# adamnelsonarcher/BB-OCR

Measured on AMD Instinct MI355X. Metric: book-page images/sec end-to-end (detect+recognize) @1280x960, higher is better.
Workload: dtype fp16

## Files before the change

### bb-ocr_amd/csrc/conv_mfma.hip

```cpp
#include "common.h"
#include "kernels.h"
#include <type_traits>
#include <utility>

__device__ __forceinline__ void lds_dma16(const void* gptr, const void* lds) {
    const unsigned la = (unsigned)(size_t)(const __attribute__((address_space(3))) void*)lds;
    asm volatile("s_mov_b32 m0, %1\n\ts_nop 0\n\tglobal_load_lds_dwordx4 %0, off" ::"v"(gptr), "s"(la) : "memory");
}

template <int EL, int MF, bool ADDUP = false>
__device__ __forceinline__ void conv_epilogue(const ConvArgs& a, f32x4 (&acc)[MF][4], int n, int nt, int oy0, int ox0, int wm, int wn, int fpr,
                                              int lane, int BN, int sub = 1, int sph = 0, int spw = 0) {
    const int g = lane >> 4, pl = lane & 15;
    const int cout0 = nt * BN + wn * 64 + g * 8;
    if (a.tail) {
        const float* tw = a.tail;
        const typename El<EL>::v8 w1f = *(const typename El<EL>::v8*)(a.tail_frag + lane * 8);
        float cb[8], b1r[4], w2a[4], w2b[4];
#pragma unroll
        for (int i = 0; i < 8; ++i) cb[i] = a.bias[(g & 1) * 8 + i];
#pragma unroll
        for (int r = 0; r < 4; ++r) { b1r[r] = tw[4 * g + r]; w2a[r] = tw[16 + 4 * g + r]; w2b[r] = tw[32 + 4 * g + r]; }
        const float b20 = tw[48], b21 = tw[49];
#pragma unroll
// ... 421 lines not shown
    const int n_wi = a.NP >> 4;
    const int l_pix = (lane & 7) + ((lane >> 5) << 3);
    const int l_kg = (lane >> 3) & 3;
    int src_pix[PITER];
#pragma unroll
    for (int it = 0; it < PITER; ++it) {
        const int wi = wave + it * NW;
        int sp = -1;
        if (wi < n_wi) {
            const int pix = wi * 16 + l_pix;
            const int py = pix / a.PW, px = pix - py * a.PW;
            const int iy = iy0 + py, ix = ix0 + px;
            if (py < a.PH && iy >= 0 && iy < a.H && ix >= 0 && ix < a.W) sp = (n * a.H + iy) * a.W + ix;
        }
        src_pix[it] = sp;
    }
    constexpr int NPART = (PITER + 3) / 4, PH = PITER / NPART;
    u32x4 pre[PH];
    auto load_part = [&](int chunk, auto part_c) {
        constexpr int part = decltype(part_c)::value;
        const int c = chunk * 32;
        const bool s0 = c < a.C0;
        const uint16_t* src = s0 ? a.in0 : a.in1;
        const int cs = s0 ? a.in0_cs : a.in1_cs;
        const int cb = (s0 ? c : c - a.C0) + l_kg * 8;
#pragma unroll
        for (int i = 0; i < PH; ++i) {
            const int sp = src_pix[part * PH + i];
            u32x4 v = {0u, 0u, 0u, 0u};
            if (sp >= 0) v = *(const u32x4*)(src + (size_t)sp * cs + cb);
            pre[i] = v;
        }
    };
    auto store_part = [&](int chunk, auto part_c) {
        constexpr int part = decltype(part_c)::value;
        unsigned char* pb = pbuf + (chunk & 1) * patch_bytes;
        const bool relu = (chunk * 32 < a.C0) ? a.relu_in0 : a.relu_in1;
#pragma unroll
        for (int i = 0; i < PH; ++i) {
            const int wi = wave + (part * PH + i) * NW;
            if (wi < n_wi) {
                u32x4 v = pre[i];
                if (relu) {
                    const s16x8 z = {0, 0, 0, 0, 0, 0, 0, 0};
                    v = __builtin_bit_cast(u32x4, __builtin_elementwise_max(__builtin_bit_cast(s16x8, v), z));
                }
                *(u32x4*)(pb + (size_t)(l_kg * a.NP + wi * 16 + l_pix) * 16) = v;
            }
        }
    };
    using P0 = std::integral_constant<int, 0>;
    const int S = (a.ntaps - 1) / NPART;
    auto stage_patch_load = [&](int chunk, int tap) {
        if (tap == 0) load_part(chunk, P0{});
        if constexpr (NPART > 1) { if (tap == S) load_part(chunk, std::integral_constant<int, (NPART > 1 ? 1 : 0)>{}); }
        if constexpr (NPART > 2) { if (tap == 2 * S) load_part(chunk, std::integral_constant<int, (NPART > 2 ? 2 : 0)>{}); }
        if constexpr (NPART > 3) { if (tap == 3 * S) load_part(chunk, std::integral_constant<int, (NPART > 3 ? 3 : 0)>{}); }
    };
    auto stage_patch_store = [&](int chunk, int tap) {
        if (tap == S - 1) store_part(chunk, P0{});
        if constexpr (NPART > 1) { if (tap == 2 * S - 1) store_part(chunk, std::integral_constant<int, (NPART > 1 ? 1 : 0)>{}); }
        if constexpr (NPART > 2) { if (tap == 3 * S - 1) store_part(chunk, std::integral_constant<int, (NPART > 2 ? 2 : 0)>{}); }
        if constexpr (NPART > 3) { if (tap == 4 * S - 1) store_part(chunk, std::integral_constant<int, (NPART > 3 ? 3 : 0)>{}); }
    };
    auto stage_patch_now = [&](int chunk) {
        load_part(chunk, P0{});
        store_part(chunk, P0{});
        if constexpr (NPART > 1) { load_part(chunk, std::integral_constant<int, (NPART > 1 ? 1 : 0)>{}); store_part(chunk, std::integral_constant<int, (NPART > 1 ? 1 : 0)>{}); }
        if constexpr (NPART > 2) { load_part(chunk, std::integral_constant<int, (NPART > 2 ? 2 : 0)>{}); store_part(chunk, std::integral_constant<int, (NPART > 2 ? 2 : 0)>{}); }
        if constexpr (NPART > 3) { load_part(chunk, std::integral_constant<int, (NPART > 3 ? 3 : 0)>{}); store_part(chunk, std::integral_constant<int, (NPART > 3 ? 3 : 0)>{}); }
    };
    const unsigned char* wsrc = (const unsigned char*)a.wpk + (size_t)nt * nk * WBUF;
    auto issue_w = [&](int ks, int buf) {
#pragma unroll
        for (int p0 = 0; p0 < WPIECES; p0 += NT) {
            if (p0 + wave * 64 < WPIECES) {
                __builtin_amdgcn_global_load_lds(
                    (const __attribute__((address_space(1))) void*)(wsrc + (size_t)ks * WBUF + (size_t)(p0 + tid) * 16),
                    (__attribute__((address_space(3))) void*)(wbuf + buf * WBUF + (p0 + wave * 64) * 16), 16, 0, 0);
            }
        }
    };

    const int fpr = a.TW >> 4;
    int frag_off[MF];
#pragma unroll
    for (int f = 0; f < MF; ++f) {
        const int F = wm * MF + f;
        const int fr = F / fpr, fc = F - fr * fpr;
        frag_off[f] = (fr * a.PW + fc * 16) * 16;
    }
    const int lane_patch_off = ((lane >> 4) * a.NP + (lane & 15)) * 16;
    const int lane_w_off = wn * 4 * 1024 + lane * 16;

    f32x4 acc[MF][4];
#pragma unroll
    for (int f = 0; f < MF; ++f)
#pragma unroll
        for (int j = 0; j < 4; ++j) acc[f][j] = (f32x4){0.f, 0.f, 0.f, 0.f};

    {
        issue_w(0, 0);
        stage_patch_now(0);
        __syncthreads();
        int ks = 0;
        for (int c = 0; c < a.nchunks; ++c) {
            const bool more = (c + 1 < a.nchunks);
            if (more && a.ntaps < 3) load_part(c + 1, P0{});
            const unsigned char* pbase = pbuf + (c & 1) * patch_bytes + lane_patch_off;
            int ky = 0, kx = 0;
            for (int tap = 0; tap < a.ntaps; ++tap, ++ks) {
                if (more && a.ntaps >= 3) stage_patch_load(c + 1, tap);
                if (ks + 1 < nk) issue_w(ks + 1, (ks + 1) & 1);
                const unsigned char* wb = wbuf + (ks & 1) * WBUF + lane_w_off;
                typename El<EL>::v8 af[4];
#pragma unroll
                for (int j = 0; j < 4; ++j) af[j] = *(const typename El<EL>::v8*)(wb + j * 1024);
                const unsigned char* pb = pbase + ((ky * a.PW + kx) * a.dil) * 16;
                typename El<EL>::v8 bq[MF];
#pragma unroll
                for (int f = 0; f < MF; ++f) bq[f] = *(const typename El<EL>::v8*)(pb + frag_off[f]);
#pragma unroll
                for (int f = 0; f < MF; ++f) {
#pragma unroll
                    for (int j = 0; j < 4; ++j) acc[f][j] = El<EL>::mfma(af[j], bq[f], acc[f][j]);
                }
                __builtin_amdgcn_sched_group_barrier(0x100, 4 + MF, 0);
                __builtin_amdgcn_sched_group_barrier(0x008, 4 * MF, 0);
                if (more) {
                    if (a.ntaps >= 3) stage_patch_store(c + 1, tap);
                    else if (tap == a.ntaps - 1) store_part(c + 1, P0{});
                }
                __syncthreads();
                if (++kx == a.KW) { kx = 0; ++ky; }
            }
        }
    }

    conv_epilogue<EL, MF>(a, acc, n, nt, oy0, ox0, wm, wn, fpr, lane, BN);
}

template <int EL, int WM, int WN, int MF, int NPB, int RING, int NPS = NPB * 64, bool FUSE1 = false, int NF = 4, int EPI = 0, int KS = 3>
__global__ void __launch_bounds__(WM * WN * 64, 2) conv3x3_dma_kernel(const ConvArgs a) {
    constexpr int NTAP = KS * KS, PAD = KS == 3 ? 1 : 0;
    static_assert((KS == 3 || KS == 2) && (KS == 3 || (!FUSE1 && EPI == 0)), "kernel size");
    constexpr int NW = WM * WN, NT = NW * 64, BN = WN * 64;
    static_assert(NW == 4, "one wave per 8-channel group of the patch");
    constexpr int WBUF = BN * 64, WPIECES = WBUF / 16, WPT = WPIECES / NT;
    static_assert(WPIECES % NT == 0 && (RING == 3 || RING == 4), "uniform DMA issue");
    constexpr int NP = NPS, PSLOTS = NTAP + 1 - RING;
    constexpr int PPER = (NPB + PSLOTS - 1) / PSLOTS;
    static_assert(NPS <= NPB * 64 && NPS > (NPB - 1) * 64 && NPS % 4 == 0, "patch size");
    static_assert(PSLOTS >= 1 && PPER * PSLOTS >= NPB, "patch does not fit the DMA schedule");
    extern __shared__ __attribute__((aligned(16))) unsigned char smem[];
    unsigned char* const wbuf = smem;
    unsigned char* const pbuf = smem + RING * WBUF;
    constexpr int patch_bytes = NP * 64;

    const int tid = threadIdx.x;
    const int lane = tid & 63;
    const int wave = __builtin_amdgcn_readfirstlane(tid >> 6);
    const int wm = wave / WN, wn = wave % WN;
    const int sub = a.sub;
    const int nk = a.nchunks * NTAP;
    const int fpr = FUSE1 ? 1 : a.TW >> 4;
    const int PW = FUSE1 ? 18 : a.PW;

    const int tile = xcd_remap(blockIdx.x, gridDim.x);
    struct Geo {
        int n, nt, oy0, ox0, sph, spw;
        const unsigned char* wsrc;
    };
    auto geom = [&](int id, Geo& g) {
        g.nt = id % a.ntiles_n;
        id /= a.ntiles_n;
        const int tx = id % a.tiles_x;
        id /= a.tiles_x;
        const int ty = id % a.tiles_y;
        int n = id / a.tiles_y;
        g.sph = 0; g.spw = 0;
        g.n = n;
        g.oy0 = ty * a.TH; g.ox0 = tx * a.TW;
        g.wsrc = (const unsigned char*)a.wpk + (size_t)g.nt * nk * WBUF;
    };
    int spix[NPB];
    const int pw_magic = (65536 + a.PW - 1) / a.PW;
    const int stack_magic = ((1 << 20) + a.stack) / (a.stack + 1);
    auto geom_pix = [&](const Geo& g) {
        const int iy0 = g.oy0 - PAD, ix0 = g.ox0 - PAD;
#pragma unroll
        for (int pb = 0; pb < NPB; ++pb) {
            const int pix = pb * 64 + lane;
            const int py = (pix * pw_magic) >> 16, px = pix - py * a.PW;
            int ly = iy0 + py;
            const int lx = ix0 + px;
            int sph = 0, spw = 0;
            bool rowok = ly >= 0;
            if (sub > 1) {
                const int vy = ly < 0 ? 0 : ly;
                const int q = (vy * stack_magic) >> 20;
                ly = vy - q * (a.stack + 1);
                sph = q / sub;
                spw = q - sph * sub;
                rowok = rowok && ly < a.stack && q < sub * sub;
            }
            const int iy = ly * sub + sph, ix = lx * sub + spw;
            spix[pb] = (py < a.PH && rowok && iy < a.H && lx >= 0 && ix < a.W) ? (g.n * a.H + iy) * a.W + ix : -1;
        }
    };
    Geo cur;
    geom(tile, cur);
    if constexpr (!FUSE1) geom_pix(cur);

    auto issue_p = [&](int sp, int chunk, int par, auto pb_c) {
        constexpr int pb = decltype(pb_c)::value;
        const int c = chunk * 32;
        const bool s0 = c < a.C0;
        const uint16_t* src = s0 ? a.in0 : a.in1;
        const int cs = s0 ? a.in0_cs : a.in1_cs;
        const int cb = (s0 ? c : c - a.C0) + wave * 8;
        const uint16_t* gp = sp >= 0 ? src + (size_t)sp * cs + cb : (const uint16_t*)a.zero;
        if ((pb + 1) * 64 <= NPS || pb * 64 + lane < NPS)
            lds_dma16(gp, pbuf + par * patch_bytes + (wave * NP + pb * 64) * 16);
    };
    auto issue_w = [&](const unsigned char* slice, int slot) {
#pragma unroll
        for (int p0 = 0; p0 < WPIECES; p0 += NT) lds_dma16(slice + (size_t)(p0 + tid) * 16, wbuf + slot * WBUF + (p0 + wave * 64) * 16);
    };
    int frag_off[MF];
#pragma unroll
    for (int f = 0; f < MF; ++f) {
        const int F = wm * MF + f;
        const int fr = F / fpr, fc = F - fr * fpr;
        frag_off[f] = (fr * PW + fc * 16) * 16;
    }
    const int lane_patch_off = ((lane >> 4) * NP + (lane & 15)) * 16;
    const int lane_w_off = wn * 4 * 1024 + lane * 16;

    struct Sched {
        static constexpr int pcnt(int tap) {
            if (FUSE1 || tap >= PSLOTS) return 0;
            const int base = NPB / PSLOTS, extra = NPB % PSLOTS;
            return base + (tap < extra ? 1 : 0);
        }
        static constexpr int pfirst(int tap) { int s = 0; for (int t = 0; t < tap; ++t) s += pcnt(t); return s; }
        static constexpr int wcnt(bool more, int tap) { return (more || tap < NTAP - (RING - 1)) ? WPT : 0; }
        static constexpr int younger(bool more, int tap) {
            int nv = wcnt(more, tap) + (more ? pcnt(tap) : 0);
            for (int back = 1; back <= RING - 2; ++back) {
                const int t = tap - back;
                const bool m = t >= 0 ? more : true;
                const int tt = t >= 0 ? t : t + NTAP;
                const int pc = m ? pcnt(tt) : 0;
                nv += (back == RING - 2) ? pc : (wcnt(m, tt) + pc);
            }
            return nv;
        }
    };
    static_assert(FUSE1 || Sched::pfirst(NTAP) == NPB, "patch DMA schedule must cover the patch");

#pragma unroll
    for (int i = 0; i < RING - 1; ++i)
        if (i < nk) issue_w(cur.wsrc + (size_t)i * WBUF, i);
    if constexpr (!FUSE1) {
        [&]<int... PB>(std::integer_sequence<int, PB...>) { (issue_p(spix[PB], 0, 0, std::integral_constant<int, PB>{}), ...); }(std::make_integer_sequence<int, NPB>{});
    } else {
        static_assert(!FUSE1 || (RING == 3 && BN == 64 && NPS == 324), "fused conv1_1 producer: 16x16 tiles, 3-deep ring of 4 KB slices");
        u32x2* const rgbp = (u32x2*)(wbuf + 2 * WBUF);
        const uint8_t* rgb = (const uint8_t*)a.in0;
        const float m0 = 0.485f * 255.0f, m1 = 0.456f * 255.0f, m2 = 0.406f * 255.0f;
        const float s0 = 0.229f * 255.0f, s1 = 0.224f * 255.0f, s2 = 0.225f * 255.0f;
        static_assert(NT == 256, "two patch pixels per thread");
        int pq[2];
        bool on_canvas[2];
        unsigned int cr[2], cg[2], cb[2];
#pragma unroll
        for (int it = 0; it < 2; ++it) {
            const int p = tid + it * NT;
            const int py = p / 20, px = p - py * 20;
            const int iy = cur.oy0 - 2 + py, ix = cur.ox0 - 2 + px;
            pq[it] = p;
            on_canvas[it] = p < 400 && iy >= 0 && iy < a.H && ix >= 0 && ix < a.W;
            const bool on_page = on_canvas[it] && iy < a.rgb_H && ix < a.rgb_W;
            const uint8_t* q = rgb + (on_page ? ((size_t)(cur.n * a.rgb_H + iy) * a.rgb_W + ix) * 3 : (size_t)cur.n * a.rgb_H * a.rgb_W * 3);
            cr[it] = q[0]; cg[it] = q[1]; cb[it] = q[2];
            if (!on_page) { cr[it] = 0u; cg[it] = 0u; cb[it] = 0u; }
        }
        typename El<EL>::v8 w1[4];
#pragma unroll
        for (int j = 0; j < 4; ++j) w1[j] = *(const typename El<EL>::v8*)(a.c11_w + ((size_t)j * 64 + lane) * 8);
        const int g = lane >> 4, pl = lane & 15;
        f32x4 b1[4];
#pragma unroll
        for (int h = 0; h < 2; ++h)
#pragma unroll
            for (int q4 = 0; q4 < 2; ++q4) b1[h * 2 + q4] = *(const f32x4*)(a.c11_b + h * 32 + g * 8 + q4 * 4);
        __builtin_amdgcn_sched_barrier(0);
#pragma unroll
        for (int it = 0; it < 2; ++it) {
            if (pq[it] < 400) {
                u32x2 v = {0u, 0u};
                if (on_canvas[it]) {
                    v[0] = El<EL>::pack2(((float)cr[it] - m0) / s0, ((float)cg[it] - m1) / s1);
                    v[1] = El<EL>::pack2(((float)cb[it] - m2) / s2, 0.f);
                }
                rgbp[pq[it]] = v;
            }
        }
        __syncthreads();
        auto frag_geo = [&](int fi, int& pp, int& py, int& px) {
            pp = fi * 16 + pl;
            py = pp / 18;
            px = pp - py * 18;
        };
#pragma unroll
        for (int b3 = 0; b3 < 2; ++b3) {
            typename El<EL>::v8 bfr[3];
            int pps[3], pys[3], pxs[3];
#pragma unroll
            for (int q = 0; q < 3; ++q) {
                const int fi = wave + (b3 * 3 + q) * NW;
                frag_geo(fi < 21 ? fi : 20, pps[q], pys[q], pxs[q]);
                const int pc = pps[q] < 324 ? pys[q] * 20 + pxs[q] : 0;
                const int t0 = 2 * g, t1 = t0 + 1;
                const u32x2 a0 = rgbp[pc + (t0 / 3) * 20 + (t0 % 3)];
                const u32x2 a1 = rgbp[pc + (t1 / 3) * 20 + (t1 % 3)];
                const u32x2 t8 = rgbp[pc + 2 * 20 + 2];
                const unsigned int x = g == 0 ? (t8[0] << 16) : (g == 1 ? (t8[1] << 16) : 0u);
                const unsigned int y = g == 0 ? (t8[0] & 0xffff0000u) : 0u;
                bfr[q] = __builtin_bit_cast(typename El<EL>::v8, (u32x4){a0[0], a0[1] | x, a1[0], a1[1] | y});
            }
            f32x4 d[3][4];
#pragma unroll
            for (int q = 0; q < 3; ++q)
#pragma unroll
                for (int j = 0; j < 4; ++j) d[q][j] = El<EL>::mfma(w1[j], bfr[q], b1[j]);
#pragma unroll
            for (int q = 0; q < 3; ++q) {
                const int fi = wave + (b3 * 3 + q) * NW;
                const int pp = pps[q];
                const int iy = cur.oy0 - 1 + pys[q], ix = cur.ox0 - 1 + pxs[q];
                const bool inside = iy >= 0 && iy < a.H && ix >= 0 && ix < a.W;
                const float cap = inside ? __builtin_inff() : 0.f;
                if (fi < 21 && pp < 324) {
#pragma unroll
                    for (int h = 0; h < 2; ++h) {
                        u32x4 o;
#pragma unroll
                        for (int i = 0; i < 4; ++i) {
                            const int k = h * 8 + i * 2;
                            const float x0 = __builtin_amdgcn_fmed3f(d[q][k >> 2][k & 3], 0.f, cap), x1 = __builtin_amdgcn_fmed3f(d[q][(k + 1) >> 2][(k + 1) & 3], 0.f, cap);
                            o[i] = El<EL>::pack2(x0, x1);
                        }
                        *(u32x4*)(pbuf + h * patch_bytes + (g * NP + pp) * 16) = o;
                    }
                }
            }
        }
    }
    asm volatile("s_waitcnt vmcnt(0) lgkmcnt(0)\n\ts_barrier" ::: "memory");

    int wslot = 0, par = 0;
    const unsigned char* wp = cur.wsrc + (size_t)(RING - 1) * WBUF;
    f32x4 acc[MF][4];
#pragma unroll
    for (int f = 0; f < MF; ++f)
#pragma unroll
        for (int j = 0; j < 4; ++j) acc[f][j] = (f32x4){0.f, 0.f, 0.f, 0.f};
    static_assert(MF % 2 == 0 && MF >= 4, "B fragments are scheduled in pairs, four ahead");
    typename El<EL>::v8 pre[4];
    auto step = [&](auto tap_c, auto more_c, int c) {
        constexpr int tap = decltype(tap_c)::value;
        constexpr bool MORE = decltype(more_c)::value;
        constexpr int ky = tap / KS, kx = tap % KS;
        const unsigned char* wb = wbuf + wslot * WBUF + lane_w_off;
        const unsigned char* pb = pbuf + par * patch_bytes + lane_patch_off + (ky * PW + kx) * 16;
        typename El<EL>::v8 af[NF], bq[MF];
#pragma unroll
        for (int j = 0; j < NF; ++j) af[j] = *(const typename El<EL>::v8*)(wb + j * 1024);
        if constexpr (tap == 0) {
#pragma unroll
            for (int f = 0; f < 4; ++f) bq[f] = *(const typename El<EL>::v8*)(pb + frag_off[f]);
        } else {
#pragma unroll
            for (int f = 0; f < 4; ++f) bq[f] = pre[f];
        }
        if constexpr (Sched::wcnt(MORE, tap) > 0) {
            int slot = wslot + RING - 1;
            if (slot >= RING) slot -= RING;
            issue_w(wp, slot);
            wp += WBUF;
        }
        if constexpr (MORE && Sched::pcnt(tap) > 0) {
            constexpr int p0 = Sched::pfirst(tap);
            const int nc = c + 1;
            [&]<int... I>(std::integer_sequence<int, I...>) { (issue_p(spix[p0 + I], nc, par ^ 1, std::integral_constant<int, p0 + I>{}), ...); }(
                std::make_integer_sequence<int, Sched::pcnt(tap)>{});
        }
        __builtin_amdgcn_sched_barrier(0);
        constexpr int kyn = (tap + 1) / KS, kxn = (tap + 1) % KS;
        const unsigned char* pbn = pbuf + par * patch_bytes + lane_patch_off + (kyn * PW + kxn) * 16;
#pragma unroll
        for (int g = 0; g < MF / 2; ++g) {
#pragma unroll
            for (int f = 2 * g; f < 2 * g + 2; ++f)
#pragma unroll
                for (int j = 0; j < NF; ++j) acc[f][j] = El<EL>::mfma(af[j], bq[f], acc[f][j]);
            __builtin_amdgcn_sched_barrier(0);
#pragma unroll
            for (int f = 2 * g + 4; f < 2 * g + 6; ++f) {
                if (f < MF) bq[f] = *(const typename El<EL>::v8*)(pb + frag_off[f]);
                else if constexpr (tap < NTAP - 1) pre[f - MF] = *(const typename El<EL>::v8*)(pbn + frag_off[f - MF]);
            }
            __builtin_amdgcn_sched_barrier(0);
        }
        asm volatile("s_waitcnt vmcnt(%0)\n\ts_barrier" ::"n"(Sched::younger(MORE, tap)) : "memory");
        wslot = wslot + 1 == RING ? 0 : wslot + 1;
    };
    auto relu_patch = [&](int c) {
        if (!((c * 32 < a.C0) ? a.relu_in0 : a.relu_in1)) return;
        const s16x8 z = {0, 0, 0, 0, 0, 0, 0, 0};
        s16x8* pp = (s16x8*)(pbuf + par * patch_bytes);
#pragma unroll
        for (int i = 0; i < (NP * 4 + NT - 1) / NT; ++i) {
            const int k = tid + i * NT;
            if ((i + 1) * NT <= NP * 4 || k < NP * 4) pp[k] = __builtin_elementwise_max(pp[k], z);
        }
        asm volatile("s_waitcnt lgkmcnt(0)\n\ts_barrier" ::: "memory");
    };
    auto chunk = [&](auto more_c, int c) {
        relu_patch(c);
        [&]<int... T>(std::integer_sequence<int, T...>) { (step(std::integral_constant<int, T>{}, more_c, c), ...); }(std::make_integer_sequence<int, NTAP>{});
        par ^= 1;
    };
    for (int c = 0; c + 1 < a.nchunks; ++c) chunk(std::true_type{}, c);
    chunk(std::false_type{}, a.nchunks - 1);
    if constexpr (FUSE1) conv_epilogue_pool2x2_lean<EL, MF>(a, acc, cur.n, cur.oy0, cur.ox0, wm, lane);
    else if constexpr (EPI == 1) conv_epilogue_post1x1<EL, MF>(a, acc, cur.n, cur.oy0, cur.ox0, wm, fpr, lane);
    else if constexpr (KS == 3 && NF == 4) {
        if (a.lean == 1) conv_epilogue_plain_lean<EL, MF>(a, acc, cur.n, cur.nt, cur.oy0, cur.ox0, wm, wn, fpr, lane, BN);
        else if (a.lean == 3) conv_epilogue_pool2x2_lean<EL, MF>(a, acc, cur.n, cur.oy0, cur.ox0, wm, lane, cur.nt * BN + wn * 64);
        else conv_epilogue<EL, MF>(a, acc, cur.n, cur.nt, cur.oy0, cur.ox0, wm, wn, fpr, lane, BN, sub, cur.sph, cur.spw);
    } else conv_epilogue<EL, MF>(a, acc, cur.n, cur.nt, cur.oy0, cur.ox0, wm, wn, fpr, lane, BN, sub, cur.sph, cur.spw);
}

template <int EL, int NCH, bool DB, int NF = 2, bool LEAN = false>
__global__ void __launch_bounds__(256, 2) conv3x3_resw_kernel(const ConvArgs a) {
    static_assert(NF == 2 || (NF == 4 && NCH == 1), "resident weights");
    constexpr int MF = 4, NP = 324, NPB = 6, NK = NCH * 9;
    constexpr int WSL = NF * 1024;
    constexpr int PCH = NP * 64;
    constexpr int NBUF = DB ? 2 : 1;
    extern __shared__ __attribute__((aligned(16))) unsigned char smem[];
    unsigned char* const wres = smem;
    unsigned char* const pbuf = smem + NK * WSL;
    const int tid = threadIdx.x, lane = tid & 63;
    const int wave = __builtin_amdgcn_readfirstlane(tid >> 6);
    const int wm = wave;
    const int ntiles = a.N * a.tiles_x * a.tiles_y;
    {
        const unsigned char* wsrc = (const unsigned char*)a.wpk;
        if constexpr (NF == 4) {
#pragma unroll
            for (int ks = 0; ks < NK; ++ks)
                __builtin_amdgcn_global_load_lds((const __attribute__((address_space(1))) void*)(wsrc + (size_t)ks * 4096 + (size_t)tid * 16),
                                                 (__attribute__((address_space(3))) void*)(wres + ks * WSL + wave * 1024), 16, 0, 0);
        } else {
#pragma unroll
            for (int k2 = 0; k2 < (NK + 1) / 2; ++k2) {
                const int ks = k2 * 2 + (tid >> 7);
                if (ks < NK)
                    __builtin_amdgcn_global_load_lds((const __attribute__((address_space(1))) void*)(wsrc + (size_t)ks * 4096 + (size_t)(tid & 127) * 16),
                                                     (__attribute__((address_space(3))) void*)(wres + (k2 * 2 + (wave >> 1)) * WSL + (wave & 1) * 1024), 16, 0, 0);
            }
        }
    }
    const int pw_magic = (65536 + 18 - 1) / 18;
    auto issue_patch = [&](int tile, int buf) {
        int id = tile;
        const int tx = id % a.tiles_x;
        id /= a.tiles_x;
        const int ty = id % a.tiles_y;
        const int n = id / a.tiles_y;
        const int iy0 = ty * 16 - 1, ix0 = tx * 16 - 1;
#pragma unroll
        for (int pb = 0; pb < NPB; ++pb) {
            const int pix = pb * 64 + lane;
            const int py = (pix * pw_magic) >> 16, px = pix - py * 18;
            const int iy = iy0 + py, ix = ix0 + px;
            const bool ok = py < 18 && iy >= 0 && iy < a.H && ix >= 0 && ix < a.W;
            const size_t sp = ((size_t)(n * a.H + iy) * a.W + ix) * a.in0_cs + wave * 8;
#pragma unroll
            for (int c = 0; c < NCH; ++c) {
                const uint16_t* gp = ok ? a.in0 + sp + c * 32 : (const uint16_t*)a.zero;
                if ((pb + 1) * 64 <= NP || pix < NP)
                    __builtin_amdgcn_global_load_lds((const __attribute__((address_space(1))) void*)gp,
                                                     (__attribute__((address_space(3))) void*)(pbuf + (buf * NCH + c) * PCH + (wave * NP + pb * 64) * 16), 16, 0, 0);
            }
        }
    };
    int frag_off[MF];
#pragma unroll
    for (int f = 0; f < MF; ++f) frag_off[f] = ((wm * MF + f) * 18) * 16;
    const int lane_patch_off = ((lane >> 4) * NP + (lane & 15)) * 16;
    const int lane_w_off = lane * 16;

    int tile = xcd_remap(blockIdx.x, gridDim.x);
    if (tile < ntiles) issue_patch(tile, 0);
    int buf = 0;
    for (; tile < ntiles; tile += gridDim.x) {
        const int next = tile + gridDim.x;
        if constexpr (DB) {
            asm volatile("s_waitcnt lgkmcnt(0)\n\ts_barrier" ::: "memory");
            if (next < ntiles) {
                issue_patch(next, buf ^ 1);
                asm volatile("s_waitcnt vmcnt(%0)\n\ts_barrier" ::"n"(NPB * NCH) : "memory");
            } else {
                asm volatile("s_waitcnt vmcnt(0)\n\ts_barrier" ::: "memory");
            }
        } else {
            asm volatile("s_waitcnt vmcnt(0)\n\ts_barrier" ::: "memory");
        }
        f32x4 acc[MF][4];
#pragma unroll
        for (int f = 0; f < MF; ++f)
#pragma unroll
            for (int j = 0; j < 4; ++j) acc[f][j] = (f32x4){0.f, 0.f, 0.f, 0.f};
#pragma unroll
        for (int c = 0; c < NCH; ++c) {
            const unsigned char* pc = pbuf + (buf * NCH + c) * PCH + lane_patch_off;
            const bool relu = a.relu_in0;
#pragma unroll
            for (int tap = 0; tap < 9; ++tap) {
                const unsigned char* wb = wres + (c * 9 + tap) * WSL + lane_w_off;
                const unsigned char* pb = pc + ((tap / 3) * 18 + (tap % 3)) * 16;
                typename El<EL>::v8 af[NF], bq[MF];
#pragma unroll
                for (int j = 0; j < NF; ++j) af[j] = *(const typename El<EL>::v8*)(wb + j * 1024);
#pragma unroll
                for (int f = 0; f < MF; ++f) bq[f] = *(const typename El<EL>::v8*)(pb + frag_off[f]);
                if (relu) {
                    const s16x8 z = {0, 0, 0, 0, 0, 0, 0, 0};
#pragma unroll
                    for (int f = 0; f < MF; ++f) bq[f] = __builtin_bit_cast(typename El<EL>::v8, __builtin_elementwise_max(__builtin_bit_cast(s16x8, bq[f]), z));
                }
#pragma unroll
                for (int f = 0; f < MF; ++f)
#pragma unroll
                    for (int j = 0; j < NF; ++j) acc[f][j] = El<EL>::mfma(af[j], bq[f], acc[f][j]);
            }
        }
        int id = tile;
        const int tx = id % a.tiles_x;
        id /= a.tiles_x;
// ... 59 lines not shown
    auto geo = [&](int oy0, int ox0, int fi) {
        Geo G;
        G.pp = fi * 16 + pl;
        const int ppc = G.pp < NP ? G.pp : NP - 1;
        const int py = ppc / 18, px = ppc - py * 18;
        const int iy = oy0 - 1 + py, ix = ox0 - 1 + px;
        G.inside = G.pp < NP && iy >= 0 && iy < a.H && ix >= 0 && ix < a.W;
        G.cy = iy < 0 ? 0 : (iy >= a.H ? a.H - 1 : iy);
        G.cx = ix < 0 ? 0 : (ix >= a.W ? a.W - 1 : ix);
        return G;
    };
    auto issue_s = [&](int n, const Geo& G, v8 (&sv)[4]) {
        const uint16_t* sp = a.in0 + ((size_t)(n * a.H + G.cy) * a.W + G.cx) * a.in0_cs + g * 8;
#pragma unroll
        for (int c = 0; c < 4; ++c) sv[c] = *(const v8*)(sp + c * 32);
    };
    auto produce = [&](int n, const Geo& G, const v8 (&sv)[4], bool more, const Geo& Gn, v8 (&sn)[4]) {
        float sy = ((float)G.cy + 0.5f) * 0.5f - 0.5f, sx = ((float)G.cx + 0.5f) * 0.5f - 0.5f;
        sy = sy < 0.f ? 0.f : sy;
        sx = sx < 0.f ? 0.f : sx;
        const int y0 = (int)sy, x0 = (int)sx;
        const int y1 = y0 + (y0 < LH - 1 ? 1 : 0), x1 = x0 + (x0 < LW - 1 ? 1 : 0);
        const float ly = sy - (float)y0, lx = sx - (float)x0, hy = 1.f - ly, hx = 1.f - lx;
        float a00 = hy * hx, a01 = hy * lx, a10 = ly * hx, a11 = ly * lx;
        asm volatile("" : "+v"(a00), "+v"(a01), "+v"(a10), "+v"(a11));
        const f32x2_t w00 = {a00, a00}, w01 = {a01, a01}, w10 = {a10, a10}, w11 = {a11, a11};
        const uint16_t* zb = a.addup + (size_t)n * LH * LW * a.up_cs + g * 8;
        const uint16_t* z00 = zb + ((size_t)y0 * LW + x0) * a.up_cs;
        const uint16_t* z01 = zb + ((size_t)y0 * LW + x1) * a.up_cs;
        const uint16_t* z10 = zb + ((size_t)y1 * LW + x0) * a.up_cs;
        const uint16_t* z11 = zb + ((size_t)y1 * LW + x1) * a.up_cs;
        u32x4 q[8];
#pragma unroll
        for (int h = 0; h < 2; ++h) {
            q[h * 4 + 0] = *(const u32x4*)(z00 + h * 32); q[h * 4 + 1] = *(const u32x4*)(z01 + h * 32);
            q[h * 4 + 2] = *(const u32x4*)(z10 + h * 32); q[h * 4 + 3] = *(const u32x4*)(z11 + h * 32);
        }
        if (more) issue_s(n, Gn, sn);
        __builtin_amdgcn_sched_barrier(0);
        f32x4 d[4];
#pragma unroll
        for (int j = 0; j < 4; ++j) d[j] = (f32x4){0.f, 0.f, 0.f, 0.f};
#pragma unroll
        for (int c = 0; c < 4; ++c)
#pragma unroll
            for (int j = 0; j < 4; ++j) d[j] = El<EL>::mfma(w1[c][j], sv[c], d[j]);

        if (G.pp < NP) {
#pragma unroll
            for (int h = 0; h < 2; ++h) {
                u32x4 o;
                const f32x4 bA = *(const f32x4*)(b1s + g * 16 + h * 8), bB = *(const f32x4*)(b1s + g * 16 + h * 8 + 4);
#pragma unroll
                for (int i = 0; i < 4; ++i) {
                    const float bk0 = i < 2 ? bA[2 * i] : bB[2 * i - 4], bk1 = i < 2 ? bA[2 * i + 1] : bB[2 * i - 3];
                    f32x2_t t = El<EL>::unpack2(q[h * 4][i]) * w00;
                    t = __builtin_elementwise_fma(El<EL>::unpack2(q[h * 4 + 1][i]), w01, t);
                    t = __builtin_elementwise_fma(El<EL>::unpack2(q[h * 4 + 2][i]), w10, t);
                    t = __builtin_elementwise_fma(El<EL>::unpack2(q[h * 4 + 3][i]), w11, t);
                    const int k = h * 8 + i * 2;
                    const float x0v = fmaxf(d[k >> 2][k & 3] + bk0 + t[0], 0.f), x1v = fmaxf(d[(k + 1) >> 2][(k + 1) & 3] + bk1 + t[1], 0.f);
                    o[i] = G.inside ? El<EL>::pack2(x0v, x1v) : 0u;
                }
                *(u32x4*)(pbuf + h * PCH + (g * NP + G.pp) * 16) = o;
            }
        }
    };
    int frag_off[MF];
#pragma unroll
    for (int f = 0; f < MF; ++f) frag_off[f] = ((wave * MF + f) * 18) * 16;
    const int lane_patch_off = (g * NP + pl) * 16;
    const int lane_w_off = lane * 16;

    for (int tile = xcd_remap(blockIdx.x, gridDim.x); tile < ntiles; tile += gridDim.x) {
        int id = tile;
        const int tx = id % a.tiles_x;
        id /= a.tiles_x;
        const int ty = id % a.tiles_y;
        const int n = id / a.tiles_y;
        const int oy0 = ty * 16, ox0 = tx * 16;
        v8 sA[4], sB[4];
        Geo G0 = geo(oy0, ox0, wave);
        issue_s(n, G0, sA);
#pragma unroll
        for (int i = 0; i < 6; ++i) {
            const int fi = wave + 4 * i;
            if (fi < NFRAG) {
                const bool more = fi + 4 < NFRAG;
                const Geo G1 = geo(oy0, ox0, more ? fi + 4 : fi);
                if (i & 1) produce(n, G0, sB, more, G1, sA);
                else produce(n, G0, sA, more, G1, sB);
                G0 = G1;
            }
        }
        asm volatile("s_waitcnt vmcnt(0) lgkmcnt(0)\n\ts_barrier" ::: "memory");
        f32x4 acc[MF][4];
#pragma unroll
        for (int f = 0; f < MF; ++f)
#pragma unroll
            for (int j = 0; j < 4; ++j) acc[f][j] = (f32x4){0.f, 0.f, 0.f, 0.f};
#pragma unroll
        for (int c = 0; c < 2; ++c) {
            const unsigned char* pc = pbuf + c * PCH + lane_patch_off;
#pragma unroll
            for (int tap = 0; tap < 9; ++tap) {
                const unsigned char* wb = wres + (c * 9 + tap) * WSL + lane_w_off;
                const unsigned char* pb = pc + ((tap / 3) * 18 + (tap % 3)) * 16;
                v8 af[NF], bq[MF];
#pragma unroll
                for (int j = 0; j < NF; ++j) af[j] = *(const v8*)(wb + j * 1024);
#pragma unroll
                for (int f = 0; f < MF; ++f) bq[f] = *(const v8*)(pb + frag_off[f]);
#pragma unroll
                for (int f = 0; f < MF; ++f)
#pragma unroll
                    for (int j = 0; j < NF; ++j) acc[f][j] = El<EL>::mfma(af[j], bq[f], acc[f][j]);
            }
        }
        asm volatile("s_waitcnt lgkmcnt(0)\n\ts_barrier" ::: "memory");
        conv_epilogue<EL, MF>(a, acc, n, 0, oy0, ox0, wave, 0, 1, lane, 64);
    }
}

template <int EL>
static hipError_t launch_up4_el(const ConvArgs& a, hipStream_t s) {
    const int ntiles = a.N * a.tiles_x * a.tiles_y;
    const int ncu = device_cus();
    const size_t smem = 18 * 2048 + 2 * 324 * 64 + 256;
    static LdsOptIn attr;
    if (hipError_t e = lds_opt_in(attr, (const void*)conv3x3_up4_kernel<EL>, smem); e != hipSuccess) return e;
    const int grid = ntiles < 2 * ncu ? ntiles : 2 * ncu;
    hipLaunchKernelGGL(conv3x3_up4_kernel<EL>, dim3(grid), dim3(256), smem, s, a);
    return hipGetLastError();
}

hipError_t launch_up4_fused(const ConvPlan& p1, const ConvPlan& p3, ConvArgs a, hipStream_t s) {
    if (p1.KH != 1 || p1.Cin != 128 || p1.Cout != 64 || p1.BN != 64 || p3.KH != 3 || p3.Cin != 64 || p3.Cout_pad != 64 || p3.BN != 64 ||
        p1.el != p3.el || p1.split || p3.split || a.in0_cs != 128 || a.up_cs != 64 || !a.addup || !a.zero || a.cout_store > 32 || (a.up_H & 1) || (a.up_W & 1) ||
        a.up_H != a.H || a.up_W != a.W)
        return hipErrorNotSupported;
    a.KH = a.KW = 3; a.pad_h = a.pad_w = 1; a.dil = 1; a.sub = 1;
    a.OH = a.H; a.OW = a.W; a.TH = a.TW = 16;
    a.tiles_x = (a.OW + 15) / 16; a.tiles_y = (a.OH + 15) / 16; a.ntiles_n = 1; a.nchunks = 2; a.ntaps = 9;
    a.aux_w = p1.d_w; a.aux_b = p1.d_b;
    a.wpk = p3.d_w; a.bias = p3.d_b;
    a.acc_scale = 1.f;
    if ((long long)a.N * a.tiles_x * a.tiles_y > 0x7fffffffLL) return hipErrorNotSupported;
    return p3.el ? launch_up4_el<1>(a, s) : launch_up4_el<0>(a, s);
}

template <int EL, int WM, int WN, int MF, int RING, bool ADDUP>
__global__ void __launch_bounds__(WM * WN * 64, (WM * WN == 8 ? 1 : 2)) conv1x1_dma_kernel(const ConvArgs a) {
    constexpr int NW = WM * WN, NT = NW * 64, BN = WN * 64;
    static_assert(NW == 4 || NW == 8, "wave w gathers channel group w & 3 of the activation tile (8 waves: half of the pixel blocks each)");
    constexpr int WBUF = BN * 64, WPIECES = WBUF / 16, WPT = WPIECES / NT;
    constexpr int NPX = WM * MF * 16, NPB = NPX / 64, PBUF = NPX * 64, SLOT = WBUF + PBUF;
    constexpr int PBW = NPB / (NW / 4);
    static_assert(WPIECES % NT == 0 && NPX % 64 == 0 && NPB % (NW / 4) == 0 && RING >= 3, "uniform DMA issue");
    extern __shared__ __attribute__((aligned(16))) unsigned char smem[];
    const int tid = threadIdx.x;
    const int lane = tid & 63;
    const int wave = __builtin_amdgcn_readfirstlane(tid >> 6);
    const int wm = wave / WN, wn = wave % WN;
    const int kg = wave & 3, pb0 = (wave >> 2) * PBW;
    int bid = xcd_remap(blockIdx.x, gridDim.x);
    const int nt = bid % a.ntiles_n;
    const int tile = bid / a.ntiles_n;
    const int px0 = tile * NPX;
    const int nk = a.nchunks;
    int pix[PBW];
#pragma unroll
    for (int i = 0; i < PBW; ++i) {
        const int p = px0 + (pb0 + i) * 64 + lane;
        pix[i] = p < a.OW ? p : -1;
    }
    const unsigned char* wsrc = (const unsigned char*)a.wpk + (size_t)nt * nk * WBUF;
    auto issue = [&](int ks, int slot) {
        unsigned char* sb = smem + slot * SLOT;
#pragma unroll
        for (int p0 = 0; p0 < WPIECES; p0 += NT) lds_dma16(wsrc + (size_t)ks * WBUF + (size_t)(p0 + tid) * 16, sb + (p0 + wave * 64) * 16);
        const int c = ks * 32;
        const bool s0 = c < a.C0;
        const uint16_t* src = s0 ? a.in0 : a.in1;
        const int cs = s0 ? a.in0_cs : a.in1_cs;
        const int cb = (s0 ? c : c - a.C0) + kg * 8;
#pragma unroll
        for (int i = 0; i < PBW; ++i) {
            const uint16_t* g = pix[i] >= 0 ? src + (size_t)pix[i] * cs + cb : (const uint16_t*)a.zero;
            lds_dma16(g, sb + WBUF + (kg * NPX + (pb0 + i) * 64) * 16);
        }
    };
    const int lane_p_off = WBUF + ((lane >> 4) * NPX + (lane & 15)) * 16 + wm * MF * 256;
    const int lane_w_off = wn * 4 * 1024 + lane * 16;
    f32x4 acc[MF][4];
#pragma unroll
    for (int f = 0; f < MF; ++f)
#pragma unroll
        for (int j = 0; j < 4; ++j) acc[f][j] = (f32x4){0.f, 0.f, 0.f, 0.f};
#pragma unroll
    for (int i = 0; i < RING - 1; ++i)
        if (i < nk) issue(i, i);
    asm volatile("s_waitcnt vmcnt(0) lgkmcnt(0)\n\ts_barrier" ::: "memory");
    int slot = 0;
    for (int ks = 0; ks < nk; ++ks) {
        const bool ahead = ks + RING - 1 < nk;
        if (ahead) {
            int sl = slot + RING - 1;
            if (sl >= RING) sl -= RING;
            issue(ks + RING - 1, sl);
        }
        const unsigned char* sb = smem + slot * SLOT;
        typename El<EL>::v8 af[4], bq[MF];
#pragma unroll
        for (int j = 0; j < 4; ++j) af[j] = *(const typename El<EL>::v8*)(sb + lane_w_off + j * 1024);
#pragma unroll
        for (int f = 0; f < MF; ++f) bq[f] = *(const typename El<EL>::v8*)(sb + lane_p_off + f * 256);
        if ((ks * 32 < a.C0) ? a.relu_in0 : a.relu_in1) {
            const s16x8 z = {0, 0, 0, 0, 0, 0, 0, 0};
#pragma unroll
            for (int f = 0; f < MF; ++f) bq[f] = __builtin_bit_cast(typename El<EL>::v8, __builtin_elementwise_max(__builtin_bit_cast(s16x8, bq[f]), z));
        }
#pragma unroll
        for (int f = 0; f < MF; ++f)
#pragma unroll
            for (int j = 0; j < 4; ++j) acc[f][j] = El<EL>::mfma(af[j], bq[f], acc[f][j]);
        if (ahead) asm volatile("s_waitcnt vmcnt(%0) lgkmcnt(0)\n\ts_barrier" ::"n"((RING - 2) * (WPT + PBW)) : "memory");
        else asm volatile("s_waitcnt vmcnt(0) lgkmcnt(0)\n\ts_barrier" ::: "memory");
        slot = slot + 1 == RING ? 0 : slot + 1;
    }
    conv_epilogue<EL, MF, ADDUP>(a, acc, 0, nt, 0, px0, wm, wn, 16, lane, BN);
}

template <int EL, int WM, int WN, int MF, bool ADDUP>
static hipError_t launch_dma1x1_k(const ConvArgs& a, long long grid, hipStream_t s) {
    constexpr int RING = 3, NPX = WM * MF * 16;
    auto k = conv1x1_dma_kernel<EL, WM, WN, MF, RING, ADDUP>;
    const size_t smem = (size_t)RING * ((size_t)WN * 64 * 64 + (size_t)NPX * 64);
    static LdsOptIn attr;
    if (hipError_t e = lds_opt_in(attr, (const void*)k, smem); e != hipSuccess) return e;
    hipLaunchKernelGGL(k, dim3((int)grid), dim3(WM * WN * 64), smem, s, a);
    return hipGetLastError();
}

template <int EL, int WM, int WN, int MF>
static hipError_t launch_dma1x1(ConvArgs a, hipStream_t s) {
    constexpr int NPX = WM * MF * 16;
    const long long total = (long long)a.N * a.H * a.W;
    if (total > 0x7fffffffLL) return hipErrorInvalidValue;
    a.N = 1; a.OH = 1; a.OW = (int)total; a.TH = 1; a.TW = NPX; a.tiles_y = 1;
    a.tiles_x = (int)((total + NPX - 1) / NPX);
    const long long grid = (long long)a.tiles_x * a.ntiles_n;
    if (grid > 0x7fffffffLL) return hipErrorInvalidValue;
    return a.addup ? launch_dma1x1_k<EL, WM, WN, MF, true>(a, grid, s) : launch_dma1x1_k<EL, WM, WN, MF, false>(a, grid, s);
}

static inline int cdiv(int a, int b) { return (a + b - 1) / b; }

size_t conv_packed_elems(const ConvPlan& p) {
    return (size_t)p.Cout_pad * p.Cin_pad * p.KH * p.KW;
}

void pack_conv_weights(const ConvPlan& p, const float* w, uint16_t* out) {
    const int BN = p.BN, ntn = p.Cout_pad / BN, nch = p.Cin_pad / 32, ntaps = p.KH * p.KW, nfr = BN / 16;
    size_t o = 0;
    for (int nt = 0; nt < ntn; ++nt)
        for (int c = 0; c < nch; ++c)
            for (int tap = 0; tap < ntaps; ++tap)
                for (int fr = 0; fr < nfr; ++fr) {
                    const int wn = fr >> 2, nf = fr & 3;
                    for (int l = 0; l < 64; ++l) {
                        const int row = l & 15;
                        const int cout = nt * BN + wn * 64 + (nf >> 1) * 32 + (row >> 2) * 8 + (nf & 1) * 4 + (row & 3);
                        for (int j = 0; j < 8; ++j) {
                            const int cin = c * 32 + 8 * (l >> 4) + j;
                            float v = 0.f;
                            if (cout < p.Cout && cin < p.Cin) v = w[((size_t)cout * p.Cin + cin) * ntaps + tap];
                            out[o++] = f32_to_el_host(p.el, v);
                        }
                    }
                }
}

template <int EL, int WM, int WN, int MF, int PITER>
static hipError_t launch_one(const ConvArgs& a, size_t smem, int grid, hipStream_t s) {
    auto k = conv_mfma_kernel<EL, WM, WN, MF, PITER>;
    static LdsOptIn attr;
    if (hipError_t e = lds_opt_in(attr, (const void*)k, smem); e != hipSuccess) return e;
    hipLaunchKernelGGL(k, dim3(grid), dim3(WM * WN * 64), smem, s, a);
    return hipGetLastError();
}

template <int EL, int WM, int WN, int MF, int PITER>
static hipError_t launch_cfg(const ConvArgs& a, int grid, hipStream_t s) {
    const size_t smem = (size_t)2 * WN * 64 * 64 + (size_t)2 * a.NP * 64;
    if (smem > 160 * 1024) return hipErrorInvalidValue;
    return launch_one<EL, WM, WN, MF, PITER>(a, smem, grid, s);
}

template <int EL, int WM, int WN, int MF, int NPB, int RING, int NPS = NPB * 64, bool FUSE1 = false, int NF = 4, int EPI = 0, int KS = 3>
static hipError_t launch_dma_one(ConvArgs a, int grid, hipStream_t s) {
    auto k = conv3x3_dma_kernel<EL, WM, WN, MF, NPB, RING, NPS, FUSE1, NF, EPI, KS>;
    const size_t smem_max = (size_t)RING * WN * 64 * 64 + (size_t)2 * NPS * 64;
    const size_t smem = (a.nchunks == 1 && !FUSE1) ? smem_max - (size_t)NPS * 64 : smem_max;
    static LdsOptIn attr;
    if (hipError_t e = lds_opt_in(attr, (const void*)k, smem_max); e != hipSuccess) return e;
    {
        a.lean = 0;
        const bool plain = !FUSE1 && EPI == 0 && KS == 3 && NF == 4 && a.sub == 1 && !a.out_f32 && !a.tail && !a.split_off && !a.addup && !a.post_w &&
                           a.acc_scale == 1.f && a.cout_store == a.ntiles_n * WN * 64 && a.out_cs % 8 == 0;
        if (plain && a.pool_mode == 0 && a.out) a.lean = 1;
        else if (plain && a.pool_mode == 1 && !a.store_full && a.TH == 16 && a.TW == 16 && a.pool_out) a.lean = 3;
    }
    hipLaunchKernelGGL(k, dim3(grid), dim3(WM * WN * 64), smem, s, a);
    return hipGetLastError();
}

template <int EL, int WM, int WN, int MF>
static hipError_t launch_dma(const ConvArgs& a, int npb, int grid, hipStream_t s) {
    if constexpr (WN == 1) {
        if (a.c11_w) {
            if (!(npb == 6 && a.PH == 18 && a.PW == 18 && a.TH == 16 && a.TW == 16 && a.nchunks == 2 && a.sub == 1)) return hipErrorInvalidValue;
            if (!(a.pool_mode == 1 && !a.store_full && !a.split_off && !a.out_f32 && !a.tail && a.cout_store == 64 && a.ntiles_n == 1 && a.acc_scale > 0.f))
                return hipErrorInvalidValue;
            return launch_dma_one<EL, WM, WN, MF, 6, 3, 324, true>(a, grid, s);
        }
    }
    if (a.post_w) {
        if constexpr (WN == 1)
            if (npb == 6 && a.PH == 18 && a.PW == 18 && a.cout_store == 64 && a.ntiles_n == 1 && a.sub == 1 && !a.pool_mode && !a.split_off &&
                !a.out_f32 && !a.tail && !a.addup)
                return launch_dma_one<EL, WM, WN, MF, 6, 3, 324, false, 4, 1>(a, grid, s);
        return hipErrorNotSupported;
    }
    if constexpr (WN == 1) {
        if (npb == 6 && a.PH * a.PW == 324) {
            if (a.cout_store <= 32 && a.nchunks <= 2 && a.sub == 1 && !a.C1 && !a.pool_mode && a.TH == 16 && a.TW == 16 && a.ntiles_n == 1)
                return launch_resw<EL>(a, s);
            if (a.cout_store == 64 && a.nchunks == 1 && a.sub == 1 && !a.C1 && a.pool_mode == 1 && !a.store_full && !a.split_off && !a.out_f32 &&
                !a.tail && !a.relu_in0 && a.TH == 16 && a.TW == 16 && a.ntiles_n == 1 && a.acc_scale > 0.f)
                return launch_resw<EL>(a, s);
            if (a.cout_store <= 32) return launch_dma_one<EL, WM, WN, MF, 6, 3, 324, false, 2>(a, grid, s);
            return launch_dma_one<EL, WM, WN, MF, 6, 3, 324>(a, grid, s);
        }
        if (npb == 6) return launch_dma_one<EL, WM, WN, MF, 6, 3>(a, grid, s);
    } else if (npb == 6) {
        const size_t wb = (size_t)WN * 64 * 64, pb = (size_t)2 * npb * 64 * 64;
        return 4 * wb + pb <= 80 * 1024 ? launch_dma_one<EL, WM, WN, MF, 6, 4>(a, grid, s) : launch_dma_one<EL, WM, WN, MF, 6, 3>(a, grid, s);
    }
    if (npb == 7) return launch_dma_one<EL, WM, WN, MF, 7, 3>(a, grid, s);
    return hipErrorInvalidValue;
}

int conv_plan_bn(int Cout) {
    return Cout > 64 ? 128 : 64;
}

template <int EL>
static hipError_t launch_conv_el(const ConvPlan& p, ConvArgs a, hipStream_t s) {
    const int BN = p.BN;
    constexpr int NWV = 4;
    constexpr int BM = 256;
    a.KH = p.KH; a.KW = p.KW; a.pad_h = p.pad_h; a.pad_w = p.pad_w; a.dil = p.dil;
    a.OH = a.H + 2 * p.pad_h - (p.KH - 1) * p.dil;
    a.OW = a.W + 2 * p.pad_w - (p.KW - 1) * p.dil;
    if (a.OH <= 0 || a.OW <= 0) return hipErrorInvalidValue;
    a.ntaps = p.KH * p.KW;
    a.sub = 1;
    if (a.post_w && !(a.zero && p.KH == 3 && p.KW == 3 && p.dil == 1 && p.pad_h == 1 && p.pad_w == 1 && BN == 64 && p.Cout_pad == 64))
        return hipErrorNotSupported;
// ... 88 lines not shown
```

Before: 967.1.

## Gather activation patches as wider per-pixel channel runs with swizzled LDS layout

The 3x3 DMA conv now has each lane pair load 32 contiguous bytes (16 channels) per pixel instead of one 16-byte channel group per wave. The 1x1 DMA conv has each group of four lanes fetch a full 64-byte pixel row of 32 channels, stored in LDS with an XOR swizzle. Patch offsets, the fused stage-1 writes and the fragment reads are remapped to match. The intent is more coalesced global loads (fewer, longer contiguous segments per pixel) and fewer LDS bank conflicts, at the cost of tighter static constraints (NPX must be 256) and more complex indexing.

```diff
diff --git a/bb-ocr_amd/csrc/conv_mfma.hip b/bb-ocr_amd/csrc/conv_mfma.hip
--- a/bb-ocr_amd/csrc/conv_mfma.hip
+++ b/bb-ocr_amd/csrc/conv_mfma.hip
@@ -597,6 +597,8 @@
     constexpr int PPER = (NPB + PSLOTS - 1) / PSLOTS;
     static_assert(NPS <= NPB * 64 && NPS > (NPB - 1) * 64 && NPS % 4 == 0, "patch size");
     static_assert(PSLOTS >= 1 && PPER * PSLOTS >= NPB, "patch does not fit the DMA schedule");
+    constexpr int NBLK = (NPS + 31) / 32;
+    static_assert(NBLK == 2 * NPB || NBLK == 2 * NPB - 1, "every wave issues NPB patch DMAs per chunk");
     extern __shared__ __attribute__((aligned(16))) unsigned char smem[];
     unsigned char* const wbuf = smem;
     unsigned char* const pbuf = smem + RING * WBUF;
@@ -628,6 +630,10 @@
         g.oy0 = ty * a.TH; g.ox0 = tx * a.TW;
         g.wsrc = (const unsigned char*)a.wpk + (size_t)g.nt * nk * WBUF;
     };
+    auto blk_of = [&](int i) {
+        const int b = 2 * i + (wave & 1);
+        return (NBLK == 2 * NPB || b < NBLK) ? b : b - 2;
+    };
     int spix[NPB];
     const int pw_magic = (65536 + a.PW - 1) / a.PW;
     const int stack_magic = ((1 << 20) + a.stack) / (a.stack + 1);
@@ -635,7 +641,7 @@
         const int iy0 = g.oy0 - PAD, ix0 = g.ox0 - PAD;
 #pragma unroll
         for (int pb = 0; pb < NPB; ++pb) {
-            const int pix = pb * 64 + lane;
+            const int pix = blk_of(pb) * 32 + (lane >> 1);
             const int py = (pix * pw_magic) >> 16, px = pix - py * a.PW;
             int ly = iy0 + py;
             const int lx = ix0 + px;
@@ -657,16 +663,18 @@
     geom(tile, cur);
     if constexpr (!FUSE1) geom_pix(cur);
 
+    const size_t lane_c8 = (lane & 1) * 8;
     auto issue_p = [&](int sp, int chunk, int par, auto pb_c) {
         constexpr int pb = decltype(pb_c)::value;
         const int c = chunk * 32;
         const bool s0 = c < a.C0;
         const uint16_t* src = s0 ? a.in0 : a.in1;
         const int cs = s0 ? a.in0_cs : a.in1_cs;
-        const int cb = (s0 ? c : c - a.C0) + wave * 8;
-        const uint16_t* gp = sp >= 0 ? src + (size_t)sp * cs + cb : (const uint16_t*)a.zero;
-        if ((pb + 1) * 64 <= NPS || pb * 64 + lane < NPS)
-            lds_dma16(gp, pbuf + par * patch_bytes + (wave * NP + pb * 64) * 16);
+        const int cb = (s0 ? c : c - a.C0) + (wave >> 1) * 16;
+        const uint16_t* gp = sp >= 0 ? (src + cb) + ((size_t)sp * cs + lane_c8) : (const uint16_t*)a.zero;
+        const int blk = blk_of(pb);
+        if (NPS % 32 == 0 || blk * 32 + (lane >> 1) < NPS)
+            lds_dma16(gp, pbuf + par * patch_bytes + (wave >> 1) * (NP * 32) + blk * 1024);
     };
     auto issue_w = [&](const unsigned char* slice, int slot) {
 #pragma unroll
@@ -677,9 +685,9 @@
     for (int f = 0; f < MF; ++f) {
         const int F = wm * MF + f;
         const int fr = F / fpr, fc = F - fr * fpr;
-        frag_off[f] = (fr * PW + fc * 16) * 16;
-    }
-    const int lane_patch_off = ((lane >> 4) * NP + (lane & 15)) * 16;
+        frag_off[f] = (fr * PW + fc * 16) * 32;
+    }
+    const int lane_patch_off = (lane >> 5) * (NP * 32) + (lane & 15) * 32 + ((lane >> 4) & 1) * 16;
     const int lane_w_off = wn * 4 * 1024 + lane * 16;
 
     struct Sched {
@@ -797,7 +805,7 @@
                             const float x0 = __builtin_amdgcn_fmed3f(d[q][k >> 2][k & 3], 0.f, cap), x1 = __builtin_amdgcn_fmed3f(d[q][(k + 1) >> 2][(k + 1) & 3], 0.f, cap);
                             o[i] = El<EL>::pack2(x0, x1);
                         }
-                        *(u32x4*)(pbuf + h * patch_bytes + (g * NP + pp) * 16) = o;
+                        *(u32x4*)(pbuf + h * patch_bytes + (g >> 1) * (NP * 32) + pp * 32 + (g & 1) * 16) = o;
                     }
                 }
             }
@@ -819,7 +827,7 @@
         constexpr bool MORE = decltype(more_c)::value;
         constexpr int ky = tap / KS, kx = tap % KS;
         const unsigned char* wb = wbuf + wslot * WBUF + lane_w_off;
-        const unsigned char* pb = pbuf + par * patch_bytes + lane_patch_off + (ky * PW + kx) * 16;
+        const unsigned char* pb = pbuf + par * patch_bytes + lane_patch_off + (ky * PW + kx) * 32;
         typename El<EL>::v8 af[NF], bq[MF];
 #pragma unroll
         for (int j = 0; j < NF; ++j) af[j] = *(const typename El<EL>::v8*)(wb + j * 1024);
@@ -844,7 +852,7 @@
         }
         __builtin_amdgcn_sched_barrier(0);
         constexpr int kyn = (tap + 1) / KS, kxn = (tap + 1) % KS;
-        const unsigned char* pbn = pbuf + par * patch_bytes + lane_patch_off + (kyn * PW + kxn) * 16;
+        const unsigned char* pbn = pbuf + par * patch_bytes + lane_patch_off + (kyn * PW + kxn) * 32;
 #pragma unroll
         for (int g = 0; g < MF / 2; ++g) {
 #pragma unroll
@@ -1210,17 +1218,18 @@
 template <int EL, int WM, int WN, int MF, int RING, bool ADDUP>
 __global__ void __launch_bounds__(WM * WN * 64, (WM * WN == 8 ? 1 : 2)) conv1x1_dma_kernel(const ConvArgs a) {
     constexpr int NW = WM * WN, NT = NW * 64, BN = WN * 64;
-    static_assert(NW == 4 || NW == 8, "wave w gathers channel group w & 3 of the activation tile (8 waves: half of the pixel blocks each)");
+    static_assert(NW == 4 || NW == 8, "wave w gathers 16 / NW of the 16-pixel blocks of the activation tile");
     constexpr int WBUF = BN * 64, WPIECES = WBUF / 16, WPT = WPIECES / NT;
     constexpr int NPX = WM * MF * 16, NPB = NPX / 64, PBUF = NPX * 64, SLOT = WBUF + PBUF;
     constexpr int PBW = NPB / (NW / 4);
-    static_assert(WPIECES % NT == 0 && NPX % 64 == 0 && NPB % (NW / 4) == 0 && RING >= 3, "uniform DMA issue");
+    static_assert(WPIECES % NT == 0 && NPX == 256 && NPB % (NW / 4) == 0 && RING >= 3, "uniform DMA issue");
     extern __shared__ __attribute__((aligned(16))) unsigned char smem[];
     const int tid = threadIdx.x;
     const int lane = tid & 63;
     const int wave = __builtin_amdgcn_readfirstlane(tid >> 6);
     const int wm = wave / WN, wn = wave % WN;
-    const int kg = wave & 3, pb0 = (wave >> 2) * PBW;
+    const size_t kg8 = ((lane & 3) ^ (((lane >> 4) & 1) * 2)) * 8;
+    const int pb0 = wave * PBW;
     int bid = xcd_remap(blockIdx.x, gridDim.x);
     const int nt = bid % a.ntiles_n;
     const int tile = bid / a.ntiles_n;
@@ -1229,7 +1238,7 @@
     int pix[PBW];
 #pragma unroll
     for (int i = 0; i < PBW; ++i) {
-        const int p = px0 + (pb0 + i) * 64 + lane;
+        const int p = px0 + (pb0 + i) * 16 + (lane >> 2);
         pix[i] = p < a.OW ? p : -1;
     }
     const unsigned char* wsrc = (const unsigned char*)a.wpk + (size_t)nt * nk * WBUF;
@@ -1241,14 +1250,14 @@
         const bool s0 = c < a.C0;
         const uint16_t* src = s0 ? a.in0 : a.in1;
         const int cs = s0 ? a.in0_cs : a.in1_cs;
-        const int cb = (s0 ? c : c - a.C0) + kg * 8;
+        const int cb = s0 ? c : c - a.C0;
 #pragma unroll
         for (int i = 0; i < PBW; ++i) {
-            const uint16_t* g = pix[i] >= 0 ? src + (size_t)pix[i] * cs + cb : (const uint16_t*)a.zero;
-            lds_dma16(g, sb + WBUF + (kg * NPX + (pb0 + i) * 64) * 16);
-        }
-    };
-    const int lane_p_off = WBUF + ((lane >> 4) * NPX + (lane & 15)) * 16 + wm * MF * 256;
+            const uint16_t* g = pix[i] >= 0 ? (src + cb) + ((size_t)(unsigned)pix[i] * (unsigned)cs + kg8) : (const uint16_t*)a.zero;
+            lds_dma16(g, sb + WBUF + (pb0 + i) * 1024);
+        }
+    };
+    const int lane_p_off = WBUF + (lane & 15) * 64 + ((lane >> 4) ^ (((lane >> 2) & 1) * 2)) * 16 + wm * MF * 1024;
     const int lane_w_off = wn * 4 * 1024 + lane * 16;
     f32x4 acc[MF][4];
 #pragma unroll
@@ -1272,7 +1281,7 @@
 #pragma unroll
         for (int j = 0; j < 4; ++j) af[j] = *(const typename El<EL>::v8*)(sb + lane_w_off + j * 1024);
 #pragma unroll
-        for (int f = 0; f < MF; ++f) bq[f] = *(const typename El<EL>::v8*)(sb + lane_p_off + f * 256);
+        for (int f = 0; f < MF; ++f) bq[f] = *(const typename El<EL>::v8*)(sb + lane_p_off + f * 1024);
         if ((ks * 32 < a.C0) ? a.relu_in0 : a.relu_in1) {
             const s16x8 z = {0, 0, 0, 0, 0, 0, 0, 0};
 #pragma unroll
```

After: 981.1 (median of 6 runs). +1.5%, better.
